# thomasahle/tinyknn

Hardware: AMD Instinct MI355X
Metric: queries/sec at Recall10@10 on GloVe-100 angular (synthetic stand-in), IVF+4-bit PQ, build_probes=1 (higher is better)
Workload: dtype int8 (saturating PQ sums) + f32 (tables, rescoring); 1 GPU; glove-100-angular stand-in: 300 Gaussian clusters sigma 0.7, N=1183514 d=100 IVF n_clusters=1087 build_probes=1 FastPQ dpb=2 M=52; k=10, n_probes=10, parallelism=replica x1 (queries sharded), batches_in_flight=2

## Files before the change

### tinyknn_amd/csrc/rescore.hip

```cpp
#include <stdlib.h>
#include <string.h>

#include <type_traits>
#include "kernels.h"

#ifndef TK_NT
#define TK_NT 0
#endif

template <typename T, typename TY>
__device__ __forceinline__ T sqdist_row(const TY *__restrict__ y, const T *xs, int d)
{
    constexpr int L = 16 / (int)sizeof(T);
    T acc[L];
#pragma unroll
    for (int l = 0; l < L; l++) acc[l] = 0;
    int i = 0;
    for (; d - i >= 4 * L; i += 4 * L) {
        T df[4 * L];
#pragma unroll
        for (int t = 0; t < 4 * L; t++) df[t] = (T)(TK_NT ? __builtin_nontemporal_load(y + i + t) : y[i + t]) - xs[i + t];
#pragma unroll
        for (int l = 0; l < L; l++) {
            T ab3 = df[3 * L + l] * df[3 * L + l] + acc[l];
            T ab2 = df[2 * L + l] * df[2 * L + l] + ab3;
            T ab1 = df[L + l] * df[L + l] + ab2;
            acc[l] = df[l] * df[l] + ab1;
        }
    }
    for (; i < d; i += L) {
#pragma unroll
        for (int l = 0; l < L; l++) {
            T df = (i + l < d) ? ((T)y[i + l] - xs[i + l]) : (T)0;
            acc[l] = df * df + acc[l];
        }
    }
    if (L == 4) return (acc[0] + acc[1]) + (acc[2 % L] + acc[3 % L]);
    return acc[0] + acc[1 % L];
}

template <typename T, typename TY, typename TX, bool DIST>
__device__ __forceinline__ void rescore_body(unsigned char *smem, const TX *__restrict__ q, int d,
                                             const TY *__restrict__ rows, int64_t n_rows,
                                             const int64_t *__restrict__ cand, int R, int k, int strip,
                                             int64_t *__restrict__ out, int *__restrict__ out_count,
                                             const TX *__restrict__ q_b, int64_t q_na, int64_t *__restrict__ out_b,
                                             int64_t out_na, T *__restrict__ out_d, T *__restrict__ out_d_b)
{
    int64_t *cs = (int64_t *)smem;
    T *ds = (T *)(smem + (size_t)R * 8);
    T *xs = ds + R;
    __shared__ int s_count;
    const int tid = threadIdx.x;
    const int64_t qi = blockIdx.x;
    const int64_t *c = cand + qi * R;

    const TX *qrow = (q_b && qi >= q_na) ? q_b + (qi - q_na) * d : q + qi * d;
    for (int t = tid; t < d; t += blockDim.x) xs[t] = (T)qrow[t];
    if (tid < 64) {
        int base = 0;
        for (int t0 = 0; t0 < R; t0 += 64) {
            int t = t0 + tid;
            int64_t id = t < R ? c[t] : -1;
            bool keep = t < R && (!strip || id != -1);
            uint64_t m = __builtin_amdgcn_ballot_w64(keep);
            int before = __builtin_popcountll(m & ((1ull << tid) - 1ull));
            if (keep) cs[base + before] = id;
            base += __builtin_popcountll(m);
        }
        if (tid == 0) s_count = base;
    }
    __syncthreads();
    const int nc = s_count;
    const bool second = out_b && qi >= out_na;
    int64_t *o = second ? out_b + (qi - out_na) * k : out + qi * k;
    T *od = nullptr;
    if (DIST) od = second ? (out_d_b ? out_d_b + (qi - out_na) * k : nullptr) : (out_d ? out_d + qi * k : nullptr);
    if (nc <= k) {
        for (int t = tid; t < k; t += blockDim.x) o[t] = t < nc ? cs[t] : -1;
        if (tid == 0 && out_count) out_count[qi] = nc;
        if (DIST && od)
            for (int t = tid; t < k; t += blockDim.x) {
                T dv = (T)__builtin_huge_valf();
                if (t < nc) {
                    int64_t id = cs[t];
                    if (id < 0) id += n_rows;
                    dv = sqdist_row<T, TY>(rows + id * (int64_t)d, xs, d);
                }
                od[t] = dv;
            }
        return;
    }
    for (int t = tid; t < nc; t += blockDim.x) {
        int64_t id = cs[t];
        if (id < 0) id += n_rows;
        if (strip & 0x100) id = 0;
        else if (strip & 0x200) id = blockIdx.x * 128 + t;
        ds[t] = sqdist_row<T, TY>(rows + id * (int64_t)d, xs, d);
    }
    __syncthreads();
    for (int t = tid; t < nc; t += blockDim.x) {
        const T dv = ds[t];
        int rank = 0;
        for (int u = 0; u < nc; u++) {
            const T du = ds[u];
            rank += (du < dv) || (du == dv && u < t);
        }
        if (rank < k) {
            o[rank] = cs[t];
            if (DIST && od) od[rank] = dv;
        }
    }
    if (tid == 0 && out_count) out_count[qi] = k;
}

template <typename T, typename TY, typename TX>
__global__ __launch_bounds__(128) void rescore_kernel(const TX *__restrict__ q, int d,
                                                      const TY *__restrict__ rows,
                                                      int64_t n_rows,
                                                      const int64_t *__restrict__ cand, int R,
                                                      int k, int strip, int64_t *__restrict__ out,
                                                      int *__restrict__ out_count, const TX *__restrict__ q_b,
                                                      int64_t q_na, int64_t *__restrict__ out_b, int64_t out_na)
{
    extern __shared__ __attribute__((aligned(16))) unsigned char smem[];
    rescore_body<T, TY, TX, false>(smem, q, d, rows, n_rows, cand, R, k, strip, out, out_count, q_b, q_na, out_b,
                                   out_na, nullptr, nullptr);
}

template <typename T, typename TY, typename TX>
__global__ __launch_bounds__(128) void rescore_dist_kernel(const TX *__restrict__ q, int d,
                                                           const TY *__restrict__ rows, int64_t n_rows,
                                                           const int64_t *__restrict__ cand, int R, int k, int strip,
                                                           int64_t *__restrict__ out, int *__restrict__ out_count,
                                                           const TX *__restrict__ q_b, int64_t q_na,
                                                           int64_t *__restrict__ out_b, int64_t out_na,
                                                           T *__restrict__ out_d, T *__restrict__ out_d_b)
{
    extern __shared__ __attribute__((aligned(16))) unsigned char smem[];
    rescore_body<T, TY, TX, true>(smem, q, d, rows, n_rows, cand, R, k, strip, out, out_count, q_b, q_na, out_b,
                                  out_na, out_d, out_d_b);
}

template <typename TY> struct RowPiece;
template <> struct RowPiece<float> { typedef float4 type; };
template <> struct RowPiece<_Float16> { typedef uint2 type; };

__device__ __forceinline__ void unpack4(const float4 p, float *o)
{
    o[0] = p.x; o[1] = p.y; o[2] = p.z; o[3] = p.w;
}

__device__ __forceinline__ void unpack4(const uint2 p, float *o)
{
    typedef _Float16 half2_t __attribute__((ext_vector_type(2)));
    const half2_t lo = __builtin_bit_cast(half2_t, p.x), hi = __builtin_bit_cast(half2_t, p.y);
    o[0] = (float)lo.x; o[1] = (float)lo.y; o[2] = (float)hi.x; o[3] = (float)hi.y;
}

template <typename P>
__device__ __forceinline__ float sqdist_row_lds(const P *__restrict__ y, const float *xs, int d)
{
    float acc[4] = {0.f, 0.f, 0.f, 0.f};
    int i = 0;
    for (; d - i >= 16; i += 16) {
        float yv[16];
        unpack4(y[(i >> 2)], yv);
        unpack4(y[(i >> 2) + 1], yv + 4);
        unpack4(y[(i >> 2) + 2], yv + 8);
        unpack4(y[(i >> 2) + 3], yv + 12);
        float df[16];
#pragma unroll
        for (int t = 0; t < 16; t++) df[t] = yv[t] - xs[i + t];
#pragma unroll
        for (int l = 0; l < 4; l++) {
            float ab3 = df[12 + l] * df[12 + l] + acc[l];
            float ab2 = df[8 + l] * df[8 + l] + ab3;
            float ab1 = df[4 + l] * df[4 + l] + ab2;
            acc[l] = df[l] * df[l] + ab1;
        }
    }
    for (; i < d; i += 4) {
        float yv[4];
        unpack4(y[i >> 2], yv);
#pragma unroll
        for (int l = 0; l < 4; l++) {
            const float df = yv[l] - xs[i + l];
            acc[l] = df * df + acc[l];
        }
    }
    return (acc[0] + acc[1]) + (acc[2] + acc[3]);
}

__device__ __forceinline__ void slots_epilogue(const TkSlotsOut &so, int64_t qi, int S, int lane, int64_t cl)
{
    const bool act = lane < S;
    bool wr = false;
    if (act && cl < 0) { cl += so.n_lists; wr = true; }
    const bool wrapped = __builtin_amdgcn_ballot_w64(wr) != 0;
    int64_t c0 = 0, rows = 0, loff = 0;
    int len = 0, n = 0;
    if (act) {
        c0 = so.list_chunk_off[cl];
        len = (int)(so.list_chunk_off[cl + 1] - c0);
        const int64_t ln = so.list_n[cl];
        n = (int)ln;
        rows = ln;
        loff = so.ids_off[cl];
    }
    int acc = len;
    int64_t racc = rows;
#pragma unroll
    for (int o = 1; o < 64; o <<= 1) {
        const int ua = __shfl_up(acc, o, 64);
        const int64_t ur = __shfl_up(racc, o, 64);
        if (lane >= o) { acc += ua; racc += ur; }
    }
    if (lane == 0) so.slot_prefix[qi * (S + 1)] = 0;
    if (act) {
        so.slot_prefix[qi * (S + 1) + lane + 1] = acc;
        so.slot_chunk0[qi * S + lane] = c0;
        so.slot_n[qi * S + lane] = n;
        so.slot_label_off[qi * S + lane] = loff;
    }
    const uint64_t full = __builtin_amdgcn_ballot_w64(act && racc >= (int64_t)so.R);
    int e = full ? __builtin_ctzll(full) + 1 : S;
    const bool plain_ok = so.slot_exact && !wrapped && so.qlim[qi] != TK_PLAIN_NEVER;
    const int e_walk = e;
    if (!plain_ok) e = S;
    bool head = false;
    if (so.slot_exact) {
        const int E = (so.R + 15) >> 4;
        const int first_len = __shfl(acc, 0, 64);
        head = plain_ok && e_walk == 1 && first_len > E;
        const int at_e = e > 0 ? __shfl(acc, e - 1, 64) : 0;
        if (lane == 0) {
            so.slot_exact[qi] = head ? 0 : e;
            so.plain0[qi] = head ? E : at_e;
        }
    }
    if (so.pair_count && act && !(so.owner && so.owner[cl] != so.me)) {
        if (head && lane == 0) {
            atomicAdd(&so.pair_count3[cl], 1);
            atomicAdd(&so.pair_count2[cl], 1);
        } else {
            atomicAdd(lane < e ? &so.pair_count[cl] : &so.pair_count2[cl], 1);
        }
    }
    if (lane == 0 && so.repeat_flag) so.repeat_flag[qi] = wrapped;
}

template <typename TY, int TILE, bool DIST>
__device__ __forceinline__ void rescore_staged_body(unsigned char *smem, const float *__restrict__ q, int d,
                                                    const TY *__restrict__ rows, int64_t n_rows,
                                                    const int64_t *__restrict__ cand, int R, int k, int strip,
                                                    int64_t *__restrict__ out, int *__restrict__ out_count,
                                                    int stride, const float *__restrict__ q_b, int64_t q_na,
                                                    int64_t *__restrict__ out_b, int64_t out_na,
                                                    const TkSlotsOut *__restrict__ so_dev, float *__restrict__ out_d,
                                                    float *__restrict__ out_d_b)
{
    typedef typename RowPiece<TY>::type P;
    const bool have_slots = so_dev != nullptr;
    int64_t *cs = (int64_t *)smem;
    float *ds = (float *)(smem + (((size_t)R * 8 + 15) & ~(size_t)15));
    float *xs = ds + ((R + 3) & ~3);
    P *tile = (P *)(xs + ((d + 3) & ~3));
    const int tid = threadIdx.x;
    const int64_t qi = blockIdx.x;
    const int64_t *c = cand + qi * R;
    const float *qrow = (q_b && qi >= q_na) ? q_b + (qi - q_na) * d : q + qi * d;
    for (int t = tid; t < d; t += 64) xs[t] = qrow[t];
    int nc = 0;
    for (int t0 = 0; t0 < R; t0 += 64) {
        const int t = t0 + tid;
        const int64_t id = t < R ? c[t] : -1;
        const bool keep = t < R && (!strip || id != -1);
        const uint64_t m = __builtin_amdgcn_ballot_w64(keep);
        const int before = __builtin_popcountll(m & ((1ull << tid) - 1ull));
        if (keep) cs[nc + before] = id;
        nc += __builtin_popcountll(m);
    }
    __syncthreads();
    const bool second = out_b && qi >= out_na;
    int64_t *o = second ? out_b + (qi - out_na) * k : out + qi * k;
    float *od = nullptr;
    if (DIST) od = second ? (out_d_b ? out_d_b + (qi - out_na) * k : nullptr) : (out_d ? out_d + qi * k : nullptr);
    if (nc <= k) {
        for (int t = tid; t < k; t += 64) o[t] = t < nc ? cs[t] : -1;
        if (tid == 0 && out_count) out_count[qi] = nc;
        if (DIST && od)
            for (int t = tid; t < k; t += 64) {
                float dv = __builtin_huge_valf();
                if (t < nc) {
                    int64_t id = cs[t];
                    if (id < 0) id += n_rows;
                    dv = sqdist_row<float, TY>(rows + id * (int64_t)d, xs, d);
                }
                od[t] = dv;
            }
        if (have_slots) slots_epilogue(*so_dev, qi, k, tid, tid < nc ? cs[tid < k ? tid : 0] : -1);
        return;
    }
    const int d4 = d >> 2;
    const int lpr_log = d4 <= 16 ? 4 : (d4 <= 32 ? 5 : 6);
    const int rr = tid >> lpr_log, pc = tid & ((1 << lpr_log) - 1), rpi = 64 >> lpr_log;
    for (int t0 = 0; t0 < nc; t0 += TILE) {
        const int nt = nc - t0 < TILE ? nc - t0 : TILE;
        if (pc < d4)
            for (int r0 = rr; r0 < nt; r0 += 16 * rpi) {
                P v[16];
#pragma unroll
                for (int u = 0; u < 16; u++) {
                    const int r = r0 + u * rpi;
                    int64_t id = cs[t0 + (r < nt ? r : nt - 1)];
                    if (id < 0) id += n_rows;
                    v[u] = ((const P *)(rows + id * (int64_t)d))[pc];
                }
#pragma unroll
                for (int u = 0; u < 16; u++) {
                    const int r = r0 + u * rpi;
                    tile[(r < nt ? r : TILE) * stride + pc] = v[u];
                }
            }
        __syncthreads();
        if (tid < nt) ds[t0 + tid] = sqdist_row_lds(tile + tid * stride, xs, d);
        __syncthreads();
    }
    constexpr int PER16 = 16 / (int)sizeof(P);
    int64_t *ps = (int64_t *)(tile + (((TILE + 1) * stride + PER16 - 1) & ~(PER16 - 1)));
    for (int t = tid; t < nc; t += 64) {
        const float dv = ds[t];
        int rank = 0;
        for (int u = 0; u < nc; u++) {
            const float du = ds[u];
            rank += (du < dv) || (du == dv && u < t);
        }
        if (rank < k) {
            o[rank] = cs[t];
            if (DIST && od) od[rank] = dv;
            if (have_slots) ps[rank] = cs[t];
        }
    }
    if (tid == 0 && out_count) out_count[qi] = k;
    if (have_slots) {
        __syncthreads();
        slots_epilogue(*so_dev, qi, k, tid, tid < k ? ps[tid] : -1);
    }
}

template <int TILE>
__global__ __launch_bounds__(64) void rescore_staged_kernel(const float *__restrict__ q, int d,
                                                            const float *__restrict__ rows,
                                                            int64_t n_rows,
                                                            const int64_t *__restrict__ cand, int R,
                                                            int k, int strip, int64_t *__restrict__ out,
                                                            int *__restrict__ out_count, int stride4,
                                                            const float *__restrict__ q_b, int64_t q_na,
                                                            int64_t *__restrict__ out_b, int64_t out_na,
                                                            const TkSlotsOut *__restrict__ so_dev)
{
    extern __shared__ __attribute__((aligned(16))) unsigned char smem[];
    rescore_staged_body<float, TILE, false>(smem, q, d, rows, n_rows, cand, R, k, strip, out, out_count, stride4, q_b,
                                            q_na, out_b, out_na, so_dev, nullptr, nullptr);
}

template <int TILE>
__global__ __launch_bounds__(64) void rescore_staged_dist_kernel(const float *__restrict__ q, int d,
                                                                 const float *__restrict__ rows, int64_t n_rows,
                                                                 const int64_t *__restrict__ cand, int R, int k,
                                                                 int strip, int64_t *__restrict__ out,
                                                                 int *__restrict__ out_count, int stride4,
                                                                 const float *__restrict__ q_b, int64_t q_na,
                                                                 int64_t *__restrict__ out_b, int64_t out_na,
                                                                 float *__restrict__ out_d, float *__restrict__ out_d_b)
{
    extern __shared__ __attribute__((aligned(16))) unsigned char smem[];
    rescore_staged_body<float, TILE, true>(smem, q, d, rows, n_rows, cand, R, k, strip, out, out_count, stride4, q_b,
                                           q_na, out_b, out_na, nullptr, out_d, out_d_b);
}

template <int TILE>
__global__ __launch_bounds__(64) void rescore_staged_half_kernel(const float *__restrict__ q, int d,
                                                                 const _Float16 *__restrict__ rows, int64_t n_rows,
                                                                 const int64_t *__restrict__ cand, int R, int k,
                                                                 int strip, int64_t *__restrict__ out,
                                                                 int *__restrict__ out_count, int stride8,
                                                                 const float *__restrict__ q_b, int64_t q_na,
                                                                 int64_t *__restrict__ out_b, int64_t out_na,
                                                                 const TkSlotsOut *__restrict__ so_dev)
{
    extern __shared__ __attribute__((aligned(16))) unsigned char smem[];
    rescore_staged_body<_Float16, TILE, false>(smem, q, d, rows, n_rows, cand, R, k, strip, out, out_count, stride8,
                                               q_b, q_na, out_b, out_na, so_dev, nullptr, nullptr);
}

template <int TILE>
__global__ __launch_bounds__(64) void rescore_staged_half_distances_kernel(const float *__restrict__ q, int d,
                                                                      const _Float16 *__restrict__ rows,
                                                                      int64_t n_rows, const int64_t *__restrict__ cand,
                                                                      int R, int k, int strip,
                                                                      int64_t *__restrict__ out,
                                                                      int *__restrict__ out_count, int stride8,
                                                                      const float *__restrict__ q_b, int64_t q_na,
                                                                      int64_t *__restrict__ out_b, int64_t out_na,
                                                                      float *__restrict__ out_d,
                                                                      float *__restrict__ out_d_b)
{
    extern __shared__ __attribute__((aligned(16))) unsigned char smem[];
    rescore_staged_body<_Float16, TILE, true>(smem, q, d, rows, n_rows, cand, R, k, strip, out, out_count, stride8,
                                              q_b, q_na, out_b, out_na, nullptr, out_d, out_d_b);
}

__global__ __launch_bounds__(128) void rescore_half_distances_kernel(const float *__restrict__ q, int d,
                                                                     const _Float16 *__restrict__ rows, int64_t n_rows,
                                                                     const int64_t *__restrict__ cand, int R, int k,
                                                                     int strip, int64_t *__restrict__ out,
                                                                     int *__restrict__ out_count,
                                                                     const float *__restrict__ q_b, int64_t q_na,
                                                                     int64_t *__restrict__ out_b, int64_t out_na,
                                                                     float *__restrict__ out_d,
                                                                     float *__restrict__ out_d_b)
{
    extern __shared__ __attribute__((aligned(16))) unsigned char smem[];
    rescore_body<float, _Float16, float, true>(smem, q, d, rows, n_rows, cand, R, k, strip, out, out_count, q_b, q_na,
                                               out_b, out_na, out_d, out_d_b);
}

struct RescoreCall {
    const void *q, *rows;
    int d, R, k, strip;
    int64_t n_rows, nq;
    const int64_t *cand;
    int64_t *out;
    int *out_count;
    hipStream_t s;
    TkSecond q2, out2;
    void *dist, *dist_b;
    bool want_d;
};

template <int TILE> static auto staged_ids_kernel(const float *) { return rescore_staged_kernel<TILE>; }
template <int TILE> static auto staged_ids_kernel(const _Float16 *) { return rescore_staged_half_kernel<TILE>; }
template <int TILE> static auto staged_dist_kernel(const float *) { return rescore_staged_dist_kernel<TILE>; }
template <int TILE> static auto staged_dist_kernel(const _Float16 *) { return rescore_staged_half_distances_kernel<TILE>; }

template <typename T, typename TY, typename TX> static auto rows_dist_kernel()
{
    if constexpr (std::is_same<TY, _Float16>::value) return rescore_half_distances_kernel;
    else return rescore_dist_kernel<T, TY, TX>;
}

template <typename T, typename TY, typename TX>
static void launch_rows(const RescoreCall &c)
{
    const dim3 grid((unsigned)c.nq), block(c.R <= 64 ? 64 : 128);
    const size_t lds = (size_t)c.R * 8 + ((size_t)c.R + c.d) * sizeof(T) + 16;
    const TX *q = (const TX *)c.q, *q_b = (const TX *)c.q2.b;
    const TY *rows = (const TY *)c.rows;
    if (c.want_d)
        hipLaunchKernelGGL((rows_dist_kernel<T, TY, TX>()), grid, block, lds, c.s, q, c.d, rows, c.n_rows, c.cand, c.R,
                           c.k, c.strip, c.out, c.out_count, q_b, c.q2.n_a, (int64_t *)c.out2.b, c.out2.n_a,
                           (T *)c.dist, (T *)c.dist_b);
    else
        hipLaunchKernelGGL((rescore_kernel<T, TY, TX>), grid, block, lds, c.s, q, c.d, rows, c.n_rows, c.cand, c.R,
                           c.k, c.strip, c.out, c.out_count, q_b, c.q2.n_a, (int64_t *)c.out2.b, c.out2.n_a);
}

template <typename TY, int TILE>
static void launch_staged_tile(const RescoreCall &c, size_t lds, int stride, const TkSlotsOut *so)
{
    const dim3 grid((unsigned)c.nq), block(64);
    const float *q = (const float *)c.q, *q_b = (const float *)c.q2.b;
    const TY *rows = (const TY *)c.rows;
    if (c.want_d)
        hipLaunchKernelGGL(staged_dist_kernel<TILE>(rows), grid, block, lds, c.s, q, c.d, rows, c.n_rows, c.cand, c.R,
                           c.k, c.strip, c.out, c.out_count, stride, q_b, c.q2.n_a, (int64_t *)c.out2.b, c.out2.n_a,
                           (float *)c.dist, (float *)c.dist_b);
    else
        hipLaunchKernelGGL(staged_ids_kernel<TILE>(rows), grid, block, lds, c.s, q, c.d, rows, c.n_rows, c.cand, c.R,
                           c.k, c.strip, c.out, c.out_count, stride, q_b, c.q2.n_a, (int64_t *)c.out2.b, c.out2.n_a,
                           so);
}

template <typename TY>
static int launch_float_sums(const RescoreCall &c, int form, const TkSlotsOut *slots)
{
    const int staged = form < 0 || form > 2 ? 2 : form;
    if (staged && c.d % 4 == 0 && c.d <= 256 && c.R <= 256) {
        const int stride = (c.d / 4) | 1;
        const int tile_rows = staged == 2 ? 32 : 64;
        const bool fuse = slots != nullptr && c.k <= 64;
        const size_t tile_bytes = (size_t)(tile_rows + 1) * stride * sizeof(typename RowPiece<TY>::type);
        const size_t lds = (((size_t)c.R * 8 + 15) & ~(size_t)15) +
                           (size_t)(((c.R + 3) & ~3) + ((c.d + 3) & ~3)) * 4 + ((tile_bytes + 15) & ~(size_t)15) +
                           (fuse ? (size_t)c.k * 8 : 0);
        if (lds <= 64 * 1024) {
            if (tile_rows == 32) launch_staged_tile<TY, 32>(c, lds, stride, fuse ? slots : nullptr);
            else launch_staged_tile<TY, 64>(c, lds, stride, fuse ? slots : nullptr);
            return fuse ? 1 : 0;
        }
    }
    launch_rows<float, TY, float>(c);
    return 0;
}

int tk_launch_rescore(const void *q, int q_is_f64, int d, const void *rows, int rows_dtype,
                      int64_t n_rows, const int64_t *cand, int R, int64_t nq, int k, int strip,
                      int64_t *out, int *out_count, hipStream_t s, int form, TkSecond q2, TkSecond out2,
                      const TkSlotsOut *slots, void *dist, TkSecond dist2)
{
    if (nq == 0 || k == 0) return 0;
    const bool want_d = dist != nullptr || dist2.b != nullptr;
    if (want_d) slots = nullptr;
    void *dist_b = out2.b ? const_cast<void *>(dist2.b) : nullptr;
    const RescoreCall c = {q, rows, d, R, k, strip, n_rows, nq, cand, out, out_count, s, q2, out2, dist, dist_b, want_d};
    if (rows_dtype == 2)
        return q_is_f64 ? -1 : launch_float_sums<_Float16>(c, form, slots);
    const int rows_is_f64 = rows_dtype == 1;
    if (!q_is_f64 && !rows_is_f64) return launch_float_sums<float>(c, form, slots);
    if (rows_is_f64 && q_is_f64) launch_rows<double, double, double>(c);
    else if (rows_is_f64) launch_rows<double, double, float>(c);
    else launch_rows<double, float, double>(c);
    return 0;
}

__global__ void make_slots_kernel(const int64_t *__restrict__ probes, int S, int64_t nq,
                                  int64_t n_lists, const int64_t *__restrict__ list_chunk_off,
                                  const int64_t *__restrict__ list_n,
                                  const int64_t *__restrict__ ids_off, int *__restrict__ slot_prefix,
                                  int64_t *__restrict__ slot_chunk0, int *__restrict__ slot_n,
                                  int64_t *__restrict__ slot_label_off,
                                  unsigned char *__restrict__ repeat_flag,
                                  int *__restrict__ pair_count, const int *__restrict__ owner,
                                  int me, const int *__restrict__ qlim, int R,
                                  int *__restrict__ slot_exact, int *__restrict__ pair_count2,
                                  int *__restrict__ plain0, int *__restrict__ pair_count3)
{
    int64_t qi = (int64_t)blockIdx.x * blockDim.x + threadIdx.x;
    if (qi >= nq) return;
    int acc = 0;
    bool wrapped = false;
    slot_prefix[qi * (S + 1)] = 0;
    int e = S;
    int64_t rows = 0;
    for (int s = 0; s < S; s++) {
        int64_t cl = probes[qi * S + s];
        if (cl < 0) { cl += n_lists; wrapped = true; }
        int64_t c0 = list_chunk_off[cl];
        acc += (int)(list_chunk_off[cl + 1] - c0);
        slot_prefix[qi * (S + 1) + s + 1] = acc;
        slot_chunk0[qi * S + s] = c0;
        slot_n[qi * S + s] = (int)list_n[cl];
        slot_label_off[qi * S + s] = ids_off[cl];
        rows += list_n[cl];
        if (e == S && rows >= (int64_t)R) e = s + 1;
    }
    const bool plain_ok = slot_exact && !wrapped && qlim[qi] != TK_PLAIN_NEVER;
    const int e_walk = e;
    if (!plain_ok) e = S;
    bool head = false;
    if (slot_exact) {
        const int E = (R + 15) >> 4;
        head = plain_ok && e_walk == 1 && slot_prefix[qi * (S + 1) + 1] > E;
        slot_exact[qi] = head ? 0 : e;
        plain0[qi] = head ? E : slot_prefix[qi * (S + 1) + e];
    }
    if (pair_count)
        for (int s = 0; s < S; s++) {
            int64_t cl = probes[qi * S + s];
            if (cl < 0) cl += n_lists;
            if (owner && owner[cl] != me) continue;
            if (head && s == 0) {
                atomicAdd(&pair_count3[cl], 1);
                atomicAdd(&pair_count2[cl], 1);
            } else {
                atomicAdd(s < e ? &pair_count[cl] : &pair_count2[cl], 1);
            }
        }
    if (repeat_flag) repeat_flag[qi] = wrapped;
}

__global__ __launch_bounds__(256) void make_slots_wave_kernel(const int64_t *__restrict__ probes, int S, int64_t nq,
                                                              const TkSlotsOut so)
{
    const int lane = threadIdx.x & 63;
    const int64_t qi = (int64_t)blockIdx.x * 4 + (threadIdx.x >> 6);
    if (qi >= nq) return;
    slots_epilogue(so, qi, S, lane, lane < S ? probes[qi * S + lane] : -1);
}

void tk_launch_make_slots(const int64_t *probes, const int *probe_count, int kc, int64_t nq,
                          int64_t n_lists, const int64_t *list_chunk_off, const int64_t *list_n,
                          const int64_t *ids_off, int *slot_prefix, int64_t *slot_chunk0,
                          int *slot_n, int64_t *slot_label_off, unsigned char *repeat_flag,
                          int *pair_count, const int *owner, int me, hipStream_t s,
                          const int *qlim, int R, int *slot_exact, int *pair_count2, int *plain0,
                          int *pair_count3)
{
    (void)probe_count;
    if (nq == 0) return;
    if (!qlim || !pair_count2 || !plain0 || !pair_count3) slot_exact = nullptr;
    if (kc <= 64 && nq >= 4096) {
        TkSlotsOut so;
        so.n_lists = n_lists; so.list_chunk_off = list_chunk_off; so.list_n = list_n; so.ids_off = ids_off;
        so.slot_prefix = slot_prefix; so.slot_chunk0 = slot_chunk0; so.slot_n = slot_n; so.slot_label_off = slot_label_off;
        so.repeat_flag = repeat_flag; so.pair_count = pair_count; so.owner = owner; so.me = me; so.qlim = qlim; so.R = R;
        so.slot_exact = slot_exact; so.pair_count2 = pair_count2; so.plain0 = plain0; so.pair_count3 = pair_count3;
        hipLaunchKernelGGL(make_slots_wave_kernel, dim3((unsigned)((nq + 3) / 4)), dim3(256), 0, s, probes, kc, nq, so);
        return;
    }
    hipLaunchKernelGGL(make_slots_kernel, dim3((unsigned)((nq + 127) / 128)), dim3(128), 0, s,
                       probes, kc, nq, n_lists, list_chunk_off, list_n, ids_off, slot_prefix,
                       slot_chunk0, slot_n, slot_label_off, repeat_flag, pair_count, owner, me,
                       qlim, R, slot_exact, pair_count2, plain0, pair_count3);
}
```

Measured before the change: 26.87 million queries/s.

## Precompute row byte offsets, pair lanes for distances, vectorize rank selection

Row byte offsets are now precomputed into LDS during compaction, so the gather loop reads them by LDS address instead of re-deriving each index. The distance pass splits every row across two lanes using float2 math and a DPP pair-sum, so all 64 lanes work instead of only the first nt. The rank selection switches to a vectorized strict-less count over registers. A check on the count sum detects ties and falls back to the original tie-breaking loop. This adds LDS use (R*16 bytes) and inline-asm address tricks, which could lower occupancy or break if the address spaces are handled wrongly.

```diff
diff --git a/tinyknn_amd/csrc/rescore.hip b/tinyknn_amd/csrc/rescore.hip
--- a/tinyknn_amd/csrc/rescore.hip
+++ b/tinyknn_amd/csrc/rescore.hip
@@ -142,54 +142,71 @@
                                   out_na, out_d, out_d_b);
 }
 
+typedef float float2_t __attribute__((ext_vector_type(2)));
+typedef float float4_t __attribute__((ext_vector_type(4)));
+typedef unsigned uint2_t __attribute__((ext_vector_type(2)));
 template <typename TY> struct RowPiece;
-template <> struct RowPiece<float> { typedef float4 type; };
-template <> struct RowPiece<_Float16> { typedef uint2 type; };
-
-__device__ __forceinline__ void unpack4(const float4 p, float *o)
-{
-    o[0] = p.x; o[1] = p.y; o[2] = p.z; o[3] = p.w;
-}
-
-__device__ __forceinline__ void unpack4(const uint2 p, float *o)
+template <> struct RowPiece<float> { typedef float4_t type; };
+template <> struct RowPiece<_Float16> { typedef uint2_t type; };
+
+template <typename P> struct HalfPiece;
+template <> struct HalfPiece<float4_t> { typedef float2_t type; };
+template <> struct HalfPiece<uint2_t> { typedef unsigned type; };
+
+__device__ __forceinline__ float2_t widen2(const float2_t p) { return p; }
+
+__device__ __forceinline__ float2_t widen2(const unsigned p)
 {
     typedef _Float16 half2_t __attribute__((ext_vector_type(2)));
-    const half2_t lo = __builtin_bit_cast(half2_t, p.x), hi = __builtin_bit_cast(half2_t, p.y);
-    o[0] = (float)lo.x; o[1] = (float)lo.y; o[2] = (float)hi.x; o[3] = (float)hi.y;
-}
-
-template <typename P>
-__device__ __forceinline__ float sqdist_row_lds(const P *__restrict__ y, const float *xs, int d)
-{
-    float acc[4] = {0.f, 0.f, 0.f, 0.f};
-    int i = 0;
-    for (; d - i >= 16; i += 16) {
-        float yv[16];
-        unpack4(y[(i >> 2)], yv);
-        unpack4(y[(i >> 2) + 1], yv + 4);
-        unpack4(y[(i >> 2) + 2], yv + 8);
-        unpack4(y[(i >> 2) + 3], yv + 12);
-        float df[16];
-#pragma unroll
-        for (int t = 0; t < 16; t++) df[t] = yv[t] - xs[i + t];
-#pragma unroll
-        for (int l = 0; l < 4; l++) {
-            float ab3 = df[12 + l] * df[12 + l] + acc[l];
-            float ab2 = df[8 + l] * df[8 + l] + ab3;
-            float ab1 = df[4 + l] * df[4 + l] + ab2;
-            acc[l] = df[l] * df[l] + ab1;
-        }
-    }
-    for (; i < d; i += 4) {
-        float yv[4];
-        unpack4(y[i >> 2], yv);
-#pragma unroll
-        for (int l = 0; l < 4; l++) {
-            const float df = yv[l] - xs[i + l];
-            acc[l] = df * df + acc[l];
-        }
-    }
-    return (acc[0] + acc[1]) + (acc[2] + acc[3]);
+    const half2_t h = __builtin_bit_cast(half2_t, p);
+    return float2_t{(float)h.x, (float)h.y};
+}
+
+template <typename H>
+__device__ __forceinline__ float sqdist_row_lds(const H *__restrict__ yp, const float2_t *xp, int d4)
+{
+    float2_t acc = {0.f, 0.f};
+    int j = 0;
+    for (; d4 - j >= 4; j += 4) {
+        float2_t df[4];
+#pragma unroll
+        for (int t = 0; t < 4; t++) df[t] = widen2(yp[2 * (j + t)]) - xp[2 * (j + t)];
+        const float2_t ab3 = df[3] * df[3] + acc;
+        const float2_t ab2 = df[2] * df[2] + ab3;
+        const float2_t ab1 = df[1] * df[1] + ab2;
+        acc = df[0] * df[0] + ab1;
+    }
+    for (; j < d4; j++) {
+        const float2_t df = widen2(yp[2 * j]) - xp[2 * j];
+        acc = df * df + acc;
+    }
+    return acc.x + acc.y;
+}
+
+#define LDS_AT(p) ((unsigned)(size_t)(__attribute__((address_space(3))) const void *)(p))
+#define LDS_PTR(T, a) ((__attribute__((address_space(3))) T *)(size_t)(a))
+#define OPAQUE(x) asm("" : "+v"(x))
+
+__device__ __forceinline__ float from_pair_lane(float v)
+{
+    return __builtin_bit_cast(float, __builtin_amdgcn_update_dpp(0, __builtin_bit_cast(int, v), 0xB1, 0xf, 0xf, false));
+}
+
+template <int NV>
+__device__ __forceinline__ void strict_counts(const float *ds, int nc4, const float *dv, int *cnt)
+{
+#pragma unroll
+    for (int j = 0; j < NV; j++) cnt[j] = 0;
+    for (int u = 0; u < nc4; u += 4) {
+        const float4_t du = *(const float4_t *)(ds + u);
+#pragma unroll
+        for (int j = 0; j < NV; j++) {
+            cnt[j] += du.x < dv[j];
+            cnt[j] += du.y < dv[j];
+            cnt[j] += du.z < dv[j];
+            cnt[j] += du.w < dv[j];
+        }
+    }
 }
 
 __device__ __forceinline__ void slots_epilogue(const TkSlotsOut &so, int64_t qi, int S, int lane, int64_t cl)
@@ -261,9 +278,11 @@
                                                     float *__restrict__ out_d_b)
 {
     typedef typename RowPiece<TY>::type P;
+    typedef typename HalfPiece<P>::type H;
     const bool have_slots = so_dev != nullptr;
     int64_t *cs = (int64_t *)smem;
-    float *ds = (float *)(smem + (((size_t)R * 8 + 15) & ~(size_t)15));
+    int64_t *ro = cs + R;
+    float *ds = (float *)(smem + (size_t)R * 16);
     float *xs = ds + ((R + 3) & ~3);
     P *tile = (P *)(xs + ((d + 3) & ~3));
     const int tid = threadIdx.x;
@@ -278,9 +297,13 @@
         const bool keep = t < R && (!strip || id != -1);
         const uint64_t m = __builtin_amdgcn_ballot_w64(keep);
         const int before = __builtin_popcountll(m & ((1ull << tid) - 1ull));
-        if (keep) cs[nc + before] = id;
+        if (keep) {
+            cs[nc + before] = id;
+            ro[nc + before] = (id < 0 ? id + n_rows : id) * (int64_t)d * (int64_t)sizeof(TY);
+        }
         nc += __builtin_popcountll(m);
     }
+    if (tid < ((-nc) & 3)) ds[nc + tid] = __builtin_huge_valf();
     __syncthreads();
     const bool second = out_b && qi >= out_na;
     int64_t *o = second ? out_b + (qi - out_na) * k : out + qi * k;
@@ -305,41 +328,75 @@
     const int d4 = d >> 2;
     const int lpr_log = d4 <= 16 ? 4 : (d4 <= 32 ? 5 : 6);
     const int rr = tid >> lpr_log, pc = tid & ((1 << lpr_log) - 1), rpi = 64 >> lpr_log;
+    const char *const lane_base = (const char *)rows + (size_t)pc * sizeof(P);
+    const unsigned ro_step = rpi * 8, st_step = rpi * stride * (unsigned)sizeof(P);
+    const int half = tid & 1, prow = tid >> 1;
+    const float2_t *const xp = (const float2_t *)xs + half;
     for (int t0 = 0; t0 < nc; t0 += TILE) {
         const int nt = nc - t0 < TILE ? nc - t0 : TILE;
         if (pc < d4)
             for (int r0 = rr; r0 < nt; r0 += 16 * rpi) {
                 P v[16];
+                unsigned ro_at = LDS_AT(ro + t0 + r0), st_at = LDS_AT(tile + r0 * stride + pc);
+                const unsigned ro_last = LDS_AT(ro + t0 + nt - 1), st_spare = LDS_AT(tile + nt * stride + pc);
+                OPAQUE(ro_at);
+                OPAQUE(st_at);
 #pragma unroll
                 for (int u = 0; u < 16; u++) {
-                    const int r = r0 + u * rpi;
-                    int64_t id = cs[t0 + (r < nt ? r : nt - 1)];
-                    if (id < 0) id += n_rows;
-                    v[u] = ((const P *)(rows + id * (int64_t)d))[pc];
+                    const unsigned a = ro_at + u * ro_step;
+                    v[u] = *(const P *)(lane_base + *LDS_PTR(const int64_t, a < ro_last ? a : ro_last));
                 }
 #pragma unroll
                 for (int u = 0; u < 16; u++) {
-                    const int r = r0 + u * rpi;
-                    tile[(r < nt ? r : TILE) * stride + pc] = v[u];
+                    const unsigned a = st_at + u * st_step;
+                    *LDS_PTR(P, a < st_spare ? a : st_spare) = v[u];
                 }
             }
         __syncthreads();
-        if (tid < nt) ds[t0 + tid] = sqdist_row_lds(tile + tid * stride, xs, d);
+        for (int rb = 0; rb < nt; rb += 32) {
+            const int r = rb + prow;
+            const float mine = sqdist_row_lds((const H *)(tile + r * stride) + half, xp, d4);
+            const float sum = mine + from_pair_lane(mine);
+            if (half == 0 && r < nt) ds[t0 + r] = sum;
+        }
         __syncthreads();
     }
     constexpr int PER16 = 16 / (int)sizeof(P);
     int64_t *ps = (int64_t *)(tile + (((TILE + 1) * stride + PER16 - 1) & ~(PER16 - 1)));
-    for (int t = tid; t < nc; t += 64) {
-        const float dv = ds[t];
-        int rank = 0;
-        for (int u = 0; u < nc; u++) {
-            const float du = ds[u];
-            rank += (du < dv) || (du == dv && u < t);
-        }
-        if (rank < k) {
-            o[rank] = cs[t];
-            if (DIST && od) od[rank] = dv;
-            if (have_slots) ps[rank] = cs[t];
+    float dv[4];
+    int cnt[4];
+#pragma unroll
+    for (int j = 0; j < 4; j++) dv[j] = tid + 64 * j < nc ? ds[tid + 64 * j] : -__builtin_huge_valf();
+    const int nc4 = (nc + 3) & ~3;
+    if (nc <= 64) { strict_counts<1>(ds, nc4, dv, cnt); cnt[1] = cnt[2] = cnt[3] = 0; }
+    else if (nc <= 128) { strict_counts<2>(ds, nc4, dv, cnt); cnt[2] = cnt[3] = 0; }
+    else strict_counts<4>(ds, nc4, dv, cnt);
+    int total = (cnt[0] + cnt[1]) + (cnt[2] + cnt[3]);
+#pragma unroll
+    for (int m = 1; m < 64; m <<= 1) total += __shfl_xor(total, m, 64);
+    if (total == nc * (nc - 1) / 2) {
+#pragma unroll
+        for (int j = 0; j < 4; j++) {
+            const int t = tid + 64 * j;
+            if (t < nc && cnt[j] < k) {
+                o[cnt[j]] = cs[t];
+                if (DIST && od) od[cnt[j]] = dv[j];
+                if (have_slots) ps[cnt[j]] = cs[t];
+            }
+        }
+    } else {
+        for (int t = tid; t < nc; t += 64) {
+            const float dvt = ds[t];
+            int rank = 0;
+            for (int u = 0; u < nc; u++) {
+                const float du = ds[u];
+                rank += (du < dvt) || (du == dvt && u < t);
+            }
+            if (rank < k) {
+                o[rank] = cs[t];
+                if (DIST && od) od[rank] = dvt;
+                if (have_slots) ps[rank] = cs[t];
+            }
         }
     }
     if (tid == 0 && out_count) out_count[qi] = k;
@@ -492,7 +549,7 @@
         const int tile_rows = staged == 2 ? 32 : 64;
         const bool fuse = slots != nullptr && c.k <= 64;
         const size_t tile_bytes = (size_t)(tile_rows + 1) * stride * sizeof(typename RowPiece<TY>::type);
-        const size_t lds = (((size_t)c.R * 8 + 15) & ~(size_t)15) +
+        const size_t lds = (size_t)c.R * 16 +
                            (size_t)(((c.R + 3) & ~3) + ((c.d + 3) & ~3)) * 4 + ((tile_bytes + 15) & ~(size_t)15) +
                            (fuse ? (size_t)c.k * 8 : 0);
         if (lds <= 64 * 1024) {
```

New measurement: 27.68 million queries/s, median of 6. 1.03x the previous value.
